# joeylitalien/drmlt-mitsuba

Hardware: AMD Instinct MI355X
Metric: mutations/sec (accepted+rejected) (higher is better)
Workload: dtype f32

## Files before the change

### drmlt-mitsuba_amd/csrc/device_path.h

```cpp
#pragma once
#include "device_bsdf.h"
#include "device_math.h"
#include "device_sampler.h"
#include "device_types.h"

struct Hit {
    int prim;
    float t, u, v;
};

typedef uint32_t u32x4_t __attribute__((ext_vector_type(4)));
template <class T> DEV T load_global16(const T *p) {
    static_assert(sizeof(T) % 16 == 0, "records are read in 16-byte words");
    typedef const u32x4_t __attribute__((address_space(1))) *GQ;
    const GQ q = (GQ) (uintptr_t) p;
    union { T v; u32x4_t w[sizeof(T) / 16]; } u;
#pragma unroll
    for (unsigned i = 0; i < sizeof(T) / 16u; ++i) u.w[i] = q[i];
    return u.v;
}
DEV f3 smooth_record_sum(const DParams &P, float index_bits, float u, float v) {
    typedef float f32x3_t __attribute__((ext_vector_type(3)));
    typedef const char __attribute__((address_space(1))) *GB;
    typedef const f32x3_t __attribute__((address_space(1))) *GQ;
// ... 296 lines not shown
    trav_run<int>(P, T, true, 0);
    return T.h;
}

typedef float float2v __attribute__((ext_vector_type(2)));
typedef const DPrimFlat __attribute__((address_space(4))) *ScalarFlatPtr;

struct FlatRec {
    float2v cx, cy, cz, cw;
    float z0, z1, z2, z3;
    int ks;
};

template <bool TRI> DEV void test_flat(const FlatRec &G, f3 o, f3 d, float tmin, float &best_t, float2v &best_uv, int &best_ks) {
    const float ldz = fmaf(G.z0, d.x, fmaf(G.z1, d.y, G.z2 * d.z));
    const float loz = fmaf(G.z0, o.x, fmaf(G.z1, o.y, fmaf(G.z2, o.z, G.z3)));
    const float t = -loz * fast_rcp(ldz);
    const float2v lo = G.cx * o.x + (G.cy * o.y + (G.cz * o.z + G.cw));
    const float2v ld = G.cx * d.x + (G.cy * d.y + G.cz * d.z);
    const float2v uv = ld * t + lo;
    float w;
    if (TRI && (G.ks & 0xff) == PRIM_TRIANGLE) w = 1.f - (uv.x + uv.y);
    else { const float2v om = 1.f - uv; w = fminf(om.x, om.y); }
    bool hit = fminf(fminf(uv.x, uv.y), w) >= 0.f && t >= tmin && t <= best_t;
    if (TRI) hit = hit && w >= 0.f;
    best_t = hit ? t : best_t;
    best_uv.x = hit ? uv.x : best_uv.x;
    best_uv.y = hit ? uv.y : best_uv.y;
    best_ks = hit ? G.ks : best_ks;
}

#define BOX_FACE_FLAG 0x40000000
typedef const DPrimBox __attribute__((address_space(4))) *ScalarBoxPtr;
struct BoxRec {
    float2v cx, cy, cz, cw;
    float z0, z1, z2, z3;
    uint32_t f0, f1, f2;
};
struct BoxCand { float t, p, q; uint32_t hc; };
DEV BoxCand box_candidate(bool leave, float nx, float ny, float fx, float fy, float tnear, float tfar, float2v lo, float2v ld, float loz, float ldz,
                          uint32_t f0, uint32_t f1, uint32_t f2) {
    BoxCand c;
    c.t = leave ? tfar : tnear;
    const float cx = leave ? fx : nx, cy = leave ? fy : ny;
    const bool a0 = cx == c.t, a1 = cy == c.t;
    const float lda = a0 ? ld.x : (a1 ? ld.y : ldz);
    const uint32_t w = a0 ? f0 : (a1 ? f1 : f2);
    c.hc = ((lda < 0.f) != leave) ? w >> 16 : w & 0xffffu;
    const float2v bxy = ld * c.t + lo;
    const float bzz = fmaf(ldz, c.t, loz);
    c.p = a0 ? bxy.y : bxy.x; c.q = (a0 || a1) ? bzz : bxy.y;
    return c;
}
DEV void test_box(const BoxRec &G, f3 o, f3 d, float tmin, float &best_t, float2v &best_uv, int &best_ks) {
    const uint32_t f0 = G.f0, f1 = G.f1, f2 = G.f2;
    const float ldz = fmaf(G.z0, d.x, fmaf(G.z1, d.y, G.z2 * d.z));
    const float loz = fmaf(G.z0, o.x, fmaf(G.z1, o.y, fmaf(G.z2, o.z, G.z3)));
    const float2v lo = G.cx * o.x + (G.cy * o.y + (G.cz * o.z + G.cw));
    const float2v ld = G.cx * d.x + (G.cy * d.y + G.cz * d.z);
    const float ix = fast_rcp(ld.x), iy = fast_rcp(ld.y), iz = fast_rcp(ldz);
    const float ax = -lo.x * ix, bx = (1.f - lo.x) * ix, ay = -lo.y * iy, by = (1.f - lo.y) * iy, az = -loz * iz, bz = (1.f - loz) * iz;
    const float nx = fminf(ax, bx), fx = fmaxf(ax, bx), ny = fminf(ay, by), fy = fmaxf(ay, by), nz = fminf(az, bz), fz = fmaxf(az, bz);
    const float tnear = fmaxf(fmaxf(nx, ny), nz), tfar = fminf(fminf(fx, fy), fz);
    const bool through = tnear <= tfar && tfar >= tmin && tnear <= best_t;
    const bool inside = !(tnear >= tmin);
    BoxCand c = box_candidate(inside, nx, ny, fx, fy, tnear, tfar, lo, ld, loz, ldz, f0, f1, f2);
    const bool hole = through && !inside && (c.hc & 1u) == 0u;
    if (__ballot(hole)) {
        const BoxCand c2 = box_candidate(true, nx, ny, fx, fy, tnear, tfar, lo, ld, loz, ldz, f0, f1, f2);
        c.t = hole ? c2.t : c.t; c.p = hole ? c2.p : c.p; c.q = hole ? c2.q : c.q; c.hc = hole ? c2.hc : c.hc;
    }
    const bool hit = through && (c.hc & 1u) != 0u && c.t >= tmin && c.t <= best_t;
    best_t = hit ? c.t : best_t;
    best_uv.x = hit ? c.p : best_uv.x;
    best_uv.y = hit ? c.q : best_uv.y;
    best_ks = hit ? (int) (c.hc | BOX_FACE_FLAG) : best_ks;
}

template <bool TRI> DEV Hit trace_flat(const DParams &P, f3 o, f3 d, float tmin, float tmax) {
    ScalarFlatPtr p = (ScalarFlatPtr) (uintptr_t) P.prims_flat;
    auto load = [](ScalarFlatPtr q, FlatRec &G) {
#ifdef DRMLT_FLAT_PLAIN_LOADS
        G.cx = float2v{q->c[0], q->c[1]}; G.cy = float2v{q->c[2], q->c[3]}; G.cz = float2v{q->c[4], q->c[5]}; G.cw = float2v{q->c[6], q->c[7]};
        G.z0 = q->rz[0]; G.z1 = q->rz[1]; G.z2 = q->rz[2]; G.z3 = q->rz[3];
        G.ks = q->kind_shade;
#else
        typedef float f8v __attribute__((ext_vector_type(8)));
        typedef float f4v __attribute__((ext_vector_type(4)));
        const f8v c = *(const volatile f8v __attribute__((address_space(4))) *) &q->c[0];
        const f4v z = *(const volatile f4v __attribute__((address_space(4))) *) &q->rz[0];
        G.ks = *(const volatile int __attribute__((address_space(4))) *) &q->kind_shade;
        G.cx = float2v{c[0], c[1]}; G.cy = float2v{c[2], c[3]}; G.cz = float2v{c[4], c[5]}; G.cw = float2v{c[6], c[7]};
        G.z0 = z[0]; G.z1 = z[1]; G.z2 = z[2]; G.z3 = z[3];
#endif
    };
#define PINF(G) asm volatile("" ::"s"(G.cx.x), "s"(G.cz.x), "s"(G.z0), "s"(G.ks))
    float best_t = tmax;
    float2v best_uv = {0.f, 0.f};
    int best_ks = -1;
    if (P.n_box > 0) {
        auto loadb = [](ScalarBoxPtr q, BoxRec &G) {
            typedef float f8v __attribute__((ext_vector_type(8)));
            typedef float f4v __attribute__((ext_vector_type(4)));
            const f8v c = *(const volatile f8v __attribute__((address_space(4))) *) &q->c[0];
            const f4v z = *(const volatile f4v __attribute__((address_space(4))) *) &q->rz[0];
            typedef const volatile uint32_t __attribute__((address_space(4))) *SU;
            G.f0 = *(SU) &q->fw[0]; G.f1 = *(SU) &q->fw[1]; G.f2 = *(SU) &q->fw[2];
            G.cx = float2v{c[0], c[1]}; G.cy = float2v{c[2], c[3]}; G.cz = float2v{c[4], c[5]}; G.cw = float2v{c[6], c[7]};
            G.z0 = z[0]; G.z1 = z[1]; G.z2 = z[2]; G.z3 = z[3];
        };
        ScalarBoxPtr pb = (ScalarBoxPtr) (uintptr_t) P.prims_box;
        BoxRec A, B;
        loadb(pb, A);
        for (int i = 0; i < P.n_box; i += 2, pb += 2) {
            asm volatile("" ::"s"(A.cx.x), "s"(A.z0), "s"(A.f0));
            loadb(pb + 1, B);
            test_box(A, o, d, tmin, best_t, best_uv, best_ks);
            if (i + 1 < P.n_box) {
                asm volatile("" ::"s"(B.cx.x), "s"(B.z0), "s"(B.f0));
                loadb(pb + 2, A);
                test_box(B, o, d, tmin, best_t, best_uv, best_ks);
            }
        }
    }
    const int n = P.n_flat_rec;
    if (n > 0) {
        FlatRec A, B;
        load(p, A);
        for (int i = 0; i < n; i += 2, p += 2) {
            PINF(A);
            load(p + 1, B);
            test_flat<TRI>(A, o, d, tmin, best_t, best_uv, best_ks);
            if (i + 1 < n) {
                PINF(B);
                load(p + 2, A);
                test_flat<TRI>(B, o, d, tmin, best_t, best_uv, best_ks);
            }
        }
    }
#undef PINF
    Hit h{-1, best_t, best_uv.x, best_uv.y};
    if (best_ks >= 0) {
        if (best_ks & BOX_FACE_FLAG) {
            const uint32_t hc = (uint32_t) best_ks & 0xffffu;
            const float uu = (hc & 2u) ? h.v : h.u, vv = (hc & 2u) ? h.u : h.v;
            h.u = (hc & 4u) ? 1.f - uu : uu;
            h.v = (hc & 8u) ? 1.f - vv : vv;
            best_ks = (int) (((hc >> 4) & 3u) | ((hc >> 6) << 8));
        }
        h.prim = best_ks >> 8;
        if ((best_ks & 0xff) == PRIM_QUAD2) {
            const bool second = h.v > h.u;
            const float uu = second ? h.u : h.u - h.v, vv = second ? h.v - h.u : h.v;
            h.prim += second ? 1 : 0;
            h.u = uu; h.v = vv;
        }
    }
    return h;
}

struct HeldScene {
    BoxRec box[3];
    FlatRec flat;
};
DEV Hit trace_held(const HeldScene &S, uint32_t n_box, uint32_t n_flat, f3 o, f3 d, float tmin, float tmax) {
    float best_t = tmax;
    float2v best_uv = {0.f, 0.f};
    int best_ks = -1;
    if (n_box > 0u) test_box(S.box[0], o, d, tmin, best_t, best_uv, best_ks);
    if (n_box > 1u) test_box(S.box[1], o, d, tmin, best_t, best_uv, best_ks);
    if (n_box > 2u) test_box(S.box[2], o, d, tmin, best_t, best_uv, best_ks);
    if (n_flat > 0u) test_flat<false>(S.flat, o, d, tmin, best_t, best_uv, best_ks);
    Hit h{-1, best_t, best_uv.x, best_uv.y};
    if (best_ks >= 0) {
        if (best_ks & BOX_FACE_FLAG) {
            const uint32_t hc = (uint32_t) best_ks & 0xffffu;
            const float uu = (hc & 2u) ? h.v : h.u, vv = (hc & 2u) ? h.u : h.v;
            h.u = (hc & 4u) ? 1.f - uu : uu;
            h.v = (hc & 8u) ? 1.f - vv : vv;
            best_ks = (int) (((hc >> 4) & 3u) | ((hc >> 6) << 8));
        }
        h.prim = best_ks >> 8;
        if ((best_ks & 0xff) == PRIM_QUAD2) {
            const bool second = h.v > h.u;
            const float uu = second ? h.u : h.u - h.v, vv = second ? h.v - h.u : h.v;
            h.prim += second ? 1 : 0;
            h.u = uu; h.v = vv;
        }
    }
    return h;
}

template <int FEAT = 15> DEV Hit trace(const DParams &P, f3 o, f3 d, float tmin, float tmax, bool any_hit) {
    if ((FEAT & 8) && P.use_bvh) return trace_bvh(P, o, d, tmin, tmax, any_hit);
    if (P.prims_flat) {
        Hit h = P.has_plain_tri ? trace_flat<true>(P, o, d, tmin, tmax) : trace_flat<false>(P, o, d, tmin, tmax);
        if (FEAT & 4)
            for (int i = P.n_flat; i < P.n_prims; ++i) {
                ScalarPrimPtr sp = (ScalarPrimPtr) (uintptr_t) P.prims;
                DPrim G;
#pragma unroll
                for (int k = 0; k < 12; ++k) G.m[k] = sp[i].m[k];
                const int ks = sp[i].kind_shade;
                G.type = PRIM_SPHERE; G.shade = ks >> 8;
                intersect_prim<4>(G, G.shade, o, d, tmin, h);
            }
        return h;
    }
    return trace_brute<FEAT>(P, o, d, tmin, tmax);
}

struct GlobalTables {
    const DShade *sh; const DBsdf *bs; const DEmitter *em;
    DEV DShade shade(int i) const { return load_global16(sh + i); }
    DEV DBsdf bsdf(int i) const { return load_global16(bs + i); }
    DEV DEmitter emitter(int i) const { return load_global16(em + i); }
    DEV float emitter_cdf_lo(int i) const { return load_global_f32(&em[i].cdf_lo); }
    DEV DShade emitter_shade(int, const DEmitter &E) const { return shade(E.prim); }
};
struct LdsTables {
    uint32_t shade_off, bsdf_off, emit_off;
    DEV DShade shade(int i) const {
        const float4 *q = reinterpret_cast<const float4 *>(&lds_x[shade_off + (uint32_t) i * 16u]);
        const float4 a = q[0], b = q[1], c = q[2], d = q[3];
        DShade s;
        s.origin[0] = a.x; s.origin[1] = a.y; s.origin[2] = a.z; s.eu[0] = a.w;
        s.eu[1] = b.x; s.eu[2] = b.y; s.ev[0] = b.z; s.ev[1] = b.w;
        s.ev[2] = c.x; s.n[0] = c.y; s.n[1] = c.z; s.n[2] = c.w;
        s.inv_len_eu = d.x; s.bsdf = __float_as_int(d.y); s.emitter = __float_as_int(d.z); s.inv_area = d.w;
        return s;
    }
    DEV DBsdf bsdf(int i) const {
        const float4 *q = reinterpret_cast<const float4 *>(&lds_x[bsdf_off + (uint32_t) i * 12u]);
        const float4 a = q[0], b = q[1], c = q[2];
        DBsdf r;
        r.type = __float_as_int(a.x); r.rgb[0] = a.y; r.rgb[1] = a.z; r.rgb[2] = a.w;
        r.p[0] = b.x; r.p[1] = b.y; r.p[2] = b.z; r.p[3] = b.w;
        r.p[4] = c.x; r.p[5] = c.y; r.p[6] = c.z; r.p[7] = c.w;
        return r;
    }
    DEV DEmitter emitter(int i) const {
        const float4 *q = reinterpret_cast<const float4 *>(&lds_x[emit_off + (uint32_t) i * 8u]);
        const float4 a = q[0], b = q[1];
        DEmitter e;
        e.radiance[0] = a.x; e.radiance[1] = a.y; e.radiance[2] = a.z; e.prim = __float_as_int(a.w);
        e.cdf_lo = b.x; e.cdf_hi = b.y; e.pad[0] = b.z; e.pad[1] = b.w;
        return e;
    }
    DEV float emitter_cdf_lo(int i) const { return lds_x[emit_off + (uint32_t) i * 8u + 4u]; }
    DEV DShade emitter_shade(int, const DEmitter &E) const { return shade(E.prim); }
    DEV int n_emitters(const DParams &P) const { return P.n_emitters; }
};
struct OneLightTables {
    LdsTables L;
    const DParams &P;
    DEV DShade shade(int i) const { return L.shade(i); }
    DEV DBsdf bsdf(int i) const { return L.bsdf(i); }
    DEV DEmitter emitter(int) const { return P.light; }
    DEV float emitter_cdf_lo(int) const { return P.light.cdf_lo; }
    DEV DShade emitter_shade(int, const DEmitter &) const { DShade s = P.light_shade; asm volatile("" : "+s"(s.inv_area)); return s; }
    DEV constexpr int n_emitters(const DParams &) const { return 1; }
};
struct HeldLightTables {
    LdsTables L;
    const DEmitter &E;
    const DShade &S;
    DEV DShade shade(int i) const { return L.shade(i); }
    DEV DBsdf bsdf(int i) const { return L.bsdf(i); }
    DEV DEmitter emitter(int) const { return E; }
    DEV float emitter_cdf_lo(int) const { return E.cdf_lo; }
    DEV DShade emitter_shade(int, const DEmitter &) const { DShade s = S; s.bsdf = __builtin_amdgcn_readfirstlane(s.bsdf); return s; }
    DEV constexpr int n_emitters(const DParams &) const { return 1; }
};
struct MixedTables {
    const DShade *sh;
    LdsTables L;
    DEV DShade shade(int i) const { return load_global16(sh + i); }
    DEV DBsdf bsdf(int i) const { return L.bsdf(i); }
    DEV DEmitter emitter(int i) const { return L.emitter(i); }
    DEV float emitter_cdf_lo(int i) const { return L.emitter_cdf_lo(i); }
    DEV DShade emitter_shade(int ei, const DEmitter &) const { return L.shade(ei); }
};
struct HybridTables {
    const DShade *sh; const DBsdf *bs; const DEmitter *em;
    LdsTables L;
    bool lds;
    DEV DShade shade(int i) const { return load_global16(sh + i); }
    DEV DBsdf bsdf(int i) const { if (lds) return L.bsdf(i); return load_global16(bs + i); }
    DEV DEmitter emitter(int i) const { if (lds) return L.emitter(i); return load_global16(em + i); }
    DEV float emitter_cdf_lo(int i) const { if (lds) return L.emitter_cdf_lo(i); return load_global_f32(&em[i].cdf_lo); }
    DEV DShade emitter_shade(int ei, const DEmitter &E) const { if (lds) return L.shade(ei); return load_global16(sh + E.prim); }
};
DEV uint32_t small_tables_floats(const DParams &P) { return (uint32_t) P.n_emitters * 16u + (uint32_t) P.n_bsdfs * 12u + (uint32_t) P.n_emitters * 8u; }
DEV void stage_bsdfs_emitters(const DParams &P, const LdsTables &T, uint32_t lane) {
    const float *src = reinterpret_cast<const float *>(P.bsdfs);
    for (uint32_t i = lane; i < (uint32_t) P.n_bsdfs * 12u; i += 64u) lds_x[T.bsdf_off + i] = src[i];
    src = reinterpret_cast<const float *>(P.emitters);
    for (uint32_t i = lane; i < (uint32_t) P.n_emitters * 8u; i += 64u) lds_x[T.emit_off + i] = src[i];
    for (uint32_t i = lane; i < (uint32_t) P.n_emitters * 16u; i += 64u) {
        const int prim = P.emitters[i >> 4].prim;
        lds_x[T.shade_off + i] = reinterpret_cast<const float *>(P.shade + prim)[i & 15u];
    }
}
DEV void stage_tables(const DParams &P, const LdsTables &T, uint32_t lane) {
    const float *src = reinterpret_cast<const float *>(P.shade);
    for (uint32_t i = lane; i < (uint32_t) P.n_shade * 16u; i += 64u) lds_x[T.shade_off + i] = src[i];
    src = reinterpret_cast<const float *>(P.bsdfs);
    for (uint32_t i = lane; i < (uint32_t) P.n_bsdfs * 12u; i += 64u) lds_x[T.bsdf_off + i] = src[i];
    src = reinterpret_cast<const float *>(P.emitters);
    for (uint32_t i = lane; i < (uint32_t) P.n_emitters * 8u; i += 64u) lds_x[T.emit_off + i] = src[i];
}

enum { PH_DONE = 0, PH_BEGIN = 1, PH_CLOSEST = 2, PH_SHADOW = 3, PH_IDLE = 4, PH_FLUSH = 5 };

struct PathState {
    f3 o, d;
    float tmin, tmax;
    f3 thr, Li;
    f3 n, s, wi;
    f3 nee;
    f3 bweight;
    float bpdf, beta_eta, eta;
    float bx, by;
    float px, py;
    int phase, depth, bsdf;
    uint32_t k;
// ... 402 lines not shown
    const float v3 = smp.next(min(k0 + 3u, kmax)), v4 = smp.next(min(k0 + 4u, kmax));
    sr.valid = false;
    f3 Li = ps.Li;
    if (ps.shadow_pending && shadow_clear) Li = Li + ps.nee;
    const bool live = ps.phase != PH_FLUSH && hit.prim >= 0;
    const DShade S = T.shade(hit.prim >= 0 ? hit.prim : 0);
    const f3 p = fma3(ld3(S.eu), hit.u, fma3(ld3(S.ev), hit.v, ld3(S.origin)));
    const f3 n = ld3(S.n);
    const f3 s = ld3(S.eu) * S.inv_len_eu;
    const bool hb = ps.has_bounce;
    const f3 thr_b = hb ? ps.thr * ps.bweight : ps.thr;
    const float eta = hb ? ps.eta * ps.beta_eta : ps.eta;
    if (!RARE_EMITTER_HIT || __ballot(live && hb && S.emitter >= 0 && ps.direct_on && ps.non_specular) != 0ull) {
        const DEmitter E = T.emitter(S.emitter >= 0 ? S.emitter : 0);
        const float dn = dot3(ps.d, n);
        const float dr = dot3(ps.d, ps.n);
        float lumPdf = S.inv_area * hit.t * hit.t / fabsf(dn);
        lumPdf *= E.cdf_hi - E.cdf_lo;
        lumPdf = (!ps.bdelta && dr >= 0.f) ? lumPdf : 0.f;
        const float a = ps.bpdf * ps.bpdf, b = lumPdf * lumPdf;
        const f3 Lm = fma3(thr_b * ld3(E.radiance), a / (a + b), Li);
        if constexpr (RARE_EMITTER_HIT) {
            const bool use = (live & hb & (S.emitter >= 0) & ps.direct_on & ps.non_specular) & (dn < 0.f);
            Li = mk3(use ? Lm.x : Li.x, use ? Lm.y : Li.y, use ? Lm.z : Li.z);
        } else
        if (live && hb && S.emitter >= 0 && ps.direct_on && ps.non_specular && dn < 0.f) Li = Lm;
    }
    const bool want_rr = hb && ps.depth >= P.rr_depth;
    const int depth = hb ? ps.depth + 1 : ps.depth;
    const bool direct_on = hb || ps.direct_on;
    const bool at_max = depth >= P.max_depth && P.max_depth > 0;
    const float rr_q = fminf(max3(thr_b) * eta * eta, 0.95f);
    const bool survives = !want_rr || !(v0 >= rr_q);
    const f3 thr = want_rr ? thr_b * (1.f / rr_q) : thr_b;
    const bool go = live && !at_max && survives;
    const f3 t = cross3(n, s);
    const f3 md = -ps.d;
    const f3 wi = mk3(dot3(md, s), dot3(md, t), dot3(md, n));
    const int bsdf = S.bsdf & 0xffffff;
    const DBsdf B = T.bsdf(bsdf);
    const bool want_nee = direct_on && B.type == 0;
    const float sx0 = want_rr ? v1 : v0, sy = want_rr ? v2 : v1;
    const int bpos = (want_rr ? 1 : 0) + (want_nee ? 2 : 0);
    const float bx = bpos == 0 ? v0 : (bpos == 1 ? v1 : (bpos == 2 ? v2 : v3));
    const float by = bpos == 0 ? v1 : (bpos == 1 ? v2 : (bpos == 2 ? v3 : v4));
    int ei = 0;
    for (int i = 1; i < T.n_emitters(P); ++i)
        if (T.emitter_cdf_lo(i) < sx0) ei = i;
    const DEmitter E = T.emitter(ei);
    const float emPdf = E.cdf_hi - E.cdf_lo;
    const float sx = (sx0 - E.cdf_lo) / emPdf;
    const DShade L = T.emitter_shade(ei, E);
    f3 lp;
    if ((L.bsdf >> 24) == PRIM_RECTANGLE) lp = fma3(ld3(L.eu), sx, fma3(ld3(L.ev), sy, ld3(L.origin)));
    else { const float a = sqrtf(fmaxf(0.f, 1.f - sx)); lp = fma3(ld3(L.eu), 1.f - a, fma3(ld3(L.ev), a * sy, ld3(L.origin))); }
    const f3 ln = ld3(L.n);
    const f3 dv = lp - p;
    const float dist2 = dot3(dv, dv), dist = sqrtf(dist2);
    const f3 dd = dv * (1.f / dist);
    const float dln = dot3(dd, ln);
    const float pdf = dln != 0.f ? L.inv_area * dist2 / fabsf(dln) : 0.f;
    const float drl = dot3(dd, n);
    const f3 wo_l = mk3(dot3(dd, s), dot3(dd, t), dot3(dd, n));
    const f3 bsdfVal = ld3(B.rgb) * (INV_PI_F * wo_l.z);
    const float bsdfPdf = INV_PI_F * wo_l.z;
    const float lpdf = pdf * emPdf;
    const float a = lpdf * lpdf, b = bsdfPdf * bsdfPdf;
    const f3 value = ld3(E.radiance) * (1.f / lpdf);
    const f3 c = thr * value * bsdfVal * (a / (a + b));
    const bool nee = go && want_nee && drl >= 0.f && dln < 0.f && pdf != 0.f && wi.z > 0.f && wo_l.z > 0.f && !is_zero3(c);
    const f3 wo = square_to_cosine_hemisphere(bx, by);
    const f3 bweight = ld3(B.rgb);
    const bool bounce = go && B.type == 0 && wi.z > 0.f && !is_zero3(bweight);
    ps.Li = Li;
    ps.k = k0 + ((live && want_rr) ? 1u : 0u) + (go ? (want_nee ? 4u : 2u) : 0u);
    ps.nrays += (nee ? 1u : 0u) + (bounce ? 1u : 0u);
    ps.shadow_pending = nee;
    ps.phase = bounce ? PH_CLOSEST : (nee ? PH_FLUSH : PH_DONE);
    if (!MASKED || nee) {
        ps.nee = c;
        sr.o = p; sr.d = dd;
        sr.tmin = ray_eps_shadow(p);
        sr.tmax = dist * (1.f - SHADOW_EPSILON_F);
        sr.valid = MASKED || nee;
    }
    if (!MASKED || bounce) {
        ps.thr = thr; ps.eta = eta; ps.depth = depth; ps.direct_on = direct_on;
        ps.wi = wi;
        ps.o = p; ps.n = n; ps.s = s;
        ps.bsdf = bsdf;
        ps.bpdf = INV_PI_F * wo.z;
        ps.bweight = bweight;
        ps.beta_eta = 1.f;
        ps.bdelta = false;
        ps.non_specular = true;
        ps.d = fma3(s, wo.x, fma3(t, wo.y, n * wo.z));
        ps.tmin = ray_eps_closest(p);
        ps.tmax = INFINITY;
        ps.has_bounce = true;
    }
}

template <class SamplerT> DEV DSplat eval_path(const DParams &P, SamplerT &smp, uint32_t &nrays, uint32_t &ndims) {
    PathState ps;
    smp.reset_caches();
    path_init(P, ps);
    Hit h{-1, 0.f, 0.f, 0.f};
// ... 16 lines not shown
```

### drmlt-mitsuba_amd/csrc/kernels.hip

```cpp
#include <algorithm>
#include <cstdlib>
#include <cstdio>
#include <type_traits>
#include "device_path.h"

#include "kernel_common.h"
#include "launch_plan.h"

__device__ __attribute__((noinline)) DSplat eval_boot_sample(const DParams &P, uint32_t index, uint32_t &nd) {
    Sampler smp;
    smp.key0 = P.key0; smp.key1 = P.key1; smp.chain = P.boot_stream; smp.major = index;
    smp.mode = SM_BOOT; smp.arr = nullptr;
    uint32_t nr;
    return eval_path(P, smp, nr, nd);
}

__global__ void __launch_bounds__(64) k_bootstrap(DParams P, uint32_t n, float *lum_out) {
    uint32_t i = blockIdx.x * blockDim.x + threadIdx.x;
    if (i >= n) return;
    uint32_t nd;
    DSplat s = eval_boot_sample(P, i, nd);
    lum_out[i] = s.lum;
    if (P.boot_weighted) { normalize_splat(s, P); lum_out[(size_t) n + i] = s.lum; }
}
// ... 821 lines not shown
#pragma unroll
    for (int i = 0; i < 12; ++i) hold_v(H.cam[i]);
#pragma unroll
    for (int i = 0; i < 3; ++i) {
        hold_v(H.light.radiance[i]); hold_v(H.light_shade.origin[i]); hold_v(H.light_shade.eu[i]); hold_v(H.light_shade.ev[i]); hold_v(H.light_shade.n[i]);
    }
    hold_v(H.light.cdf_lo); hold_v(H.light.cdf_hi); hold_v(H.light_shade.inv_area); hold_v(H.light_shade.bsdf);
}
DEV RowSamplerT<RULE_ORBITAL> w2_sampler(uint32_t key0, uint32_t key1) {
    RowSamplerT<RULE_ORBITAL> s;
    s.key0 = key0; s.key1 = key1;
    s.mode = SM_STAGE1; s.type = 2; s.sigma2 = 0.f;
    s.stride = V4_STRIDE;
    s.x_off = s.y_off = s.xyz = 0u;
    return s;
}
template <bool BOX> DEV void w2_film_put_channel(const DParams &P, const float *lut, float px, float py, float v, int ch) {
    if (P.debug & 1) return;
    float posx = px - 0.5f, posy = py - 0.5f;
    int minx = max((int) ceilf(posx - P.filter_radius), 0), miny = max((int) ceilf(posy - P.filter_radius), 0);
    int maxx = min((int) floorf(posx + P.filter_radius), P.width - 1), maxy = min((int) floorf(posy + P.filter_radius), P.height - 1);
    for (int y = miny; y <= maxy; ++y) {
        const int iy = min((int) fabsf(((float) y - posy) * P.filter_scale), 31);
        float wy = BOX ? (iy < 31 ? P.box_weight : 0.f) : lut[iy];
        for (int x = minx; x <= maxx; ++x) {
            const int ix = min((int) fabsf(((float) x - posx) * P.filter_scale), 31);
            float w = (BOX ? (ix < 31 ? P.box_weight : 0.f) : lut[ix]) * wy;
            atomic_add_global_f32(P.film + ((size_t) y * P.width + x) * 3 + ch, w * v);
        }
    }
}
template <bool BOX> DEV void w2_flush_passes(const DParams &P, const V4Lds &L, const float *lut, uint32_t qn, uint32_t lane) {
    const uint32_t s = lane / 3u, ch = lane - 3u * s;
    for (uint32_t base = 0u; base < qn; base += 21u) {
        const uint32_t e = base + s;
        if (e < qn && s < 21u) {
            const float *q = &lds_x[L.q_off + e];
            w2_film_put_channel<BOX>(P, lut, q[0], q[L.qcap], q[(2u + ch) * L.qcap], (int) ch);
        }
    }
}
DEV void w2_flush(const DParams &P, const V4Lds &L, uint32_t &qn, uint32_t lane) {
    float *const lut = &lds_x[L.list_off];
    if (P.box_weight > 0.f) w2_flush_passes<true>(P, L, lut, qn, lane);
    else if (qn) {
        if (lane < 32u) lut[lane] = P.filter_lut[lane];
        w2_flush_passes<false>(P, L, lut, qn, lane);
    }
    qn = 0u;
}

struct W2HeldScene {
    HeldScene S;
    uint32_t counts;
};
struct W2StreamedScene {};
template <class Rec> DEV void w2_hold_rows(Rec &G, const float *c, const float *rz, bool have) {
    float v[12];
#pragma unroll
    for (int k = 0; k < 12; ++k) v[k] = 0.f;
    if (have) {
#pragma unroll
        for (int k = 0; k < 8; ++k) v[k] = c[k];
#pragma unroll
        for (int k = 0; k < 4; ++k) v[8 + k] = rz[k];
    }
#pragma unroll
    for (int k = 0; k < 12; ++k) hold_v(v[k]);
    G.cx = float2v{v[0], v[1]}; G.cy = float2v{v[2], v[3]}; G.cz = float2v{v[4], v[5]}; G.cw = float2v{v[6], v[7]};
    G.z0 = v[8]; G.z1 = v[9]; G.z2 = v[10]; G.z3 = v[11];
}
DEV W2HeldScene w2_held_scene(const DParams &P) {
    W2HeldScene H;
    const uint32_t n_box = (uint32_t) min(max(P.n_box, 0), 3), n_flat = (uint32_t) min(max(P.n_flat_rec, 0), 1);
#pragma unroll
    for (uint32_t i = 0; i < 3u; ++i) {
        BoxRec &G = H.S.box[i];
        const DPrimBox *q = P.prims_box + i;
        w2_hold_rows(G, q->c, q->rz, i < n_box);
        uint32_t f0 = 0u, f1 = 0u, f2 = 0u;
        if (i < n_box) { f0 = q->fw[0]; f1 = q->fw[1]; f2 = q->fw[2]; }
        hold_v(f0); hold_v(f1); hold_v(f2);
        G.f0 = f0; G.f1 = f1; G.f2 = f2;
    }
    FlatRec &F = H.S.flat;
    w2_hold_rows(F, P.prims_flat->c, P.prims_flat->rz, n_flat > 0u);
    int ks = -1;
    if (n_flat > 0u) ks = P.prims_flat->kind_shade;
    hold_v(ks);
    F.ks = ks;
    H.counts = n_box | (n_flat << 8);
    hold_v(H.counts);
    return H;
}

template <bool HELD> __global__ void __launch_bounds__(CHAIN_BLOCK, 2) k_mutate_w2(DParams P, uint32_t n_mut, uint32_t mut_base) {
    typedef RowSamplerT<RULE_ORBITAL> RowSampler;
    if (threadIdx.x == 0) {
        atomicAdd(P.stats + 14, 1ull); atomicAdd(P.stats + 15, 1ull); atomicAdd(P.stats + 16, 1ull);
        if constexpr (HELD) atomicAdd(P.stats + 17, 1ull);
    }
    const uint32_t lane = threadIdx.x;
    const uint32_t sub = lane & 31u;
    const bool helper = lane >= 32u;
    const uint32_t c = blockIdx.x * 32u + sub;
    const bool live = !helper && c < P.n_chains;
    const uint32_t cc = c < P.n_chains ? c : P.n_chains - 1;
    const uint32_t S = V4_STRIDE;
    int smp_mode = SM_STAGE1;
    uint32_t roles;
    uint32_t qn = 0u;
    ChainState cs;
    float cum = 0.f;
    Counters ct = {0u, 0u, 0u, 0u, 0u};
    PathState ps;
    bool helper_has_ray = false;
    Hit h{-1, 0.f, 0.f, 0.f};
    int batch;
    uint32_t base = 0u, target = 0u, limit = 0u;
    bool reported = false;
    W2Held held = w2_held(P);
    w2_hold(held);
    typename std::conditional<HELD, W2HeldScene, W2StreamedScene>::type scene;
    if constexpr (HELD) scene = w2_held_scene(P);
    uint32_t imp_lo = (uint32_t) (uintptr_t) P.importance, imp_hi = (uint32_t) ((uintptr_t) P.importance >> 32);
    uint32_t done_lo = (uint32_t) (uintptr_t) P.chain_done, done_hi = (uint32_t) ((uintptr_t) P.chain_done >> 32);
    uint32_t left_lo = (uint32_t) (uintptr_t) P.waves_left, left_hi = (uint32_t) ((uintptr_t) P.waves_left >> 32);
    uint32_t key0_v = P.key0, key1_v = P.key1, chain_off_v = P.chain_offset, timid_v = (uint32_t) P.timid_after_large;
    hold_v(imp_lo); hold_v(imp_hi); hold_v(done_lo); hold_v(done_hi); hold_v(left_lo); hold_v(left_hi);
    hold_v(key0_v); hold_v(key1_v); hold_v(chain_off_v); hold_v(timid_v);
    {
        const V4Layout<RULE_ORBITAL> Y = v4_layout<RULE_ORBITAL>(P, V4_QCAP);
        roles = RowSampler::first_roles(Y.group, sub);
        if (!helper) {
            for (uint32_t k = 0; k < Y.D; ++k) lds_x[k * S + sub] = unwrap01(P.x[(size_t) k * P.n_chains + cc]);
            for (uint32_t k = Y.D; k < Y.D4; ++k) lds_x[k * S + sub] = 0.f;
        }
        cs.cur.lum = P.cur_lum[cc]; cs.cur.px = P.cur_px[cc]; cs.cur.py = P.cur_py[cc];
        cs.cur.r = P.cur_r[cc]; cs.cur.g = P.cur_g[cc]; cs.cur.b = P.cur_b[cc];
        cs.y = cs.cur; cs.z = cs.cur;
        cs.a1 = 0.f; cs.coin_acc1 = cs.coin_acc2 = cs.coin_mix = 0.f;
        cs.it = 0u; cs.nd1 = cs.nd2 = 0u; cs.stage = -1; cs.large = false;
        path_init(P, ps);
        base = (P.chain_done && live) ? P.chain_done[cc] : mut_base;
        target = P.chain_done ? n_mut : mut_base + n_mut;
// ... 120 lines not shown
                        const uint32_t ii = valid ? i : 0u;
                        const uint32_t b = (uint32_t) (((float) ii + 0.5f) * rcp_n), j = ii - b * n;
                        const uint32_t cj = (uint32_t) lds_list[j];
                        const uint32_t mj = (uint32_t) __shfl((int) maj_mine, (int) cj, 64);
                        const unsigned inf = (unsigned) __shfl((int) info, (int) cj, 64);
                        smg.set_roles(inf, C.group, cj);
                        const bool coin = b >= nb1;
                        if (valid) {
                            const u4 r = philox4x32_10(Pm.key0, Pm.key1, coin ? 0u : b, coin ? mj + 1u : mj, chain_base_g + cj, coin ? TAG_COIN : TAG_S1);
                            const Unit4 u{{u32_to_unit(r.x), u32_to_unit(r.y), u32_to_unit(r.z), u32_to_unit(r.w)}};
                            if (!coin) row_fill_first_drawn(smg, b, u, (inf & 1u) != 0u);
                            else {
                                float *dst = &lds_x[L.coin_off + cj];
                                dst[0] = u.v[0]; dst[S] = u.v[1]; dst[2u * S] = u.v[2]; dst[3u * S] = u.v[3];
                            }
                        }
                    }
                }
                const uint32_t f2mask = (uint32_t) __ballot(kind == 2);
                if (f2mask) {
                    if (kind == 2) lds_list[__builtin_amdgcn_mbcnt_lo(f2mask, 0u)] = (int) sub;
                    const uint32_t nb2 = Pm.timid_after_large ? D4 / 4u : (D4 / 2u + 3u) / 4u;
                    const uint32_t n = (uint32_t) __popc(f2mask), total = n * nb2;
                    const float rcp_n = 1.f / (float) n;
                    for (uint32_t fb = 0u; fb < total; fb += 64u) {
                        const uint32_t i = fb + lane;
                        const bool valid = i < total;
                        const uint32_t ii = valid ? i : 0u;
                        const uint32_t b = (uint32_t) (((float) ii + 0.5f) * rcp_n), j = ii - b * n;
                        const uint32_t cj = (uint32_t) lds_list[j];
                        const uint32_t mj = (uint32_t) __shfl((int) maj_mine, (int) cj, 64);
                        const unsigned inf = (unsigned) __shfl((int) info, (int) cj, 64);
                        smg.set_roles(inf, C.group, cj);
                        if (valid) smg.fill_second(b, D4, mj, chain_base_g + cj, (inf & 1u) != 0u);
                    }
                }
            }

            if (parked) {
                if (kind == 0) ps.phase = PH_IDLE;
                else {
                    DParams Vb{};
                    Vb.exclude_direct = C.exclude_direct; Vb.width = C.width; Vb.height = C.height;
                    Vb.tan_half_fov = C.tan_half_fov; Vb.inv_aspect = C.inv_aspect; Vb.near_clip = C.near_clip; Vb.far_clip = C.far_clip;
#pragma unroll
                    for (int q = 0; q < 12; ++q) Vb.cam[q] = C.cam[q];
                    smp_mode = smp.mode = cs.stage == 0 ? SM_STAGE1 : SM_STAGE2;
                    path_init(Vb, ps);
                    const float v0 = smp.next(0u), v1 = smp.next(1u);
                    path_begin(Vb, ps, v0, v1);
                }
            }
        }
        const bool tracing = helper ? helper_has_ray : ps.phase == PH_CLOSEST;
        __builtin_amdgcn_s_setprio(0);
        if constexpr (HELD) {
            if (__ballot(tracing)) {
                const uint32_t counts = wave_uniform(scene.counts);
                h = trace_held(scene.S, counts & 0xffu, counts >> 8, ps.o, ps.d, ps.tmin, ps.tmax);
            }
        } else {
            SECTION_PARAMS(Pt);
            if (__ballot(tracing)) h = trace<0>(Pt, ps.o, ps.d, ps.tmin, ps.tmax, helper);
        }
        __builtin_amdgcn_s_setprio(3);
        const unsigned occluded = from_upper_u((helper_has_ray && h.prim >= 0) ? 1u : 0u);
        helper_has_ray = false;
        ShadowRay sr;
        asm volatile("" : "=v"(sr.d.x), "=v"(sr.d.y), "=v"(sr.d.z), "=v"(sr.tmin), "=v"(sr.tmax));
        sr.o = ps.o; sr.valid = false;
        {
            const W2Held &Cs = held;
            if (!helper && ps.phase != PH_DONE && ps.phase != PH_IDLE) {
                RowSampler sms = w2_sampler(0u, 0u);
                sms.set_roles(roles, Cs.group, sub); sms.mode = smp_mode;
                DParams Vs{};
                Vs.eff_dim = Cs.eff_dim; Vs.rr_depth = Cs.rr_depth; Vs.max_depth = Cs.max_depth;
                const LdsTables LT{Cs.shade_off, Cs.bsdf_off, 0u};
                path_step_diffuse<RowSampler, HeldLightTables, false, HELD>(Vs, HeldLightTables{LT, Cs.light, Cs.light_shade}, ps, sms, h, occluded == 0u, sr);
            }
        }
        ps.o.x = lower_keeps(ps.o.x, sr.o.x); ps.o.y = lower_keeps(ps.o.y, sr.o.y); ps.o.z = lower_keeps(ps.o.z, sr.o.z);
        ps.d.x = lower_keeps(ps.d.x, sr.d.x); ps.d.y = lower_keeps(ps.d.y, sr.d.y); ps.d.z = lower_keeps(ps.d.z, sr.d.z);
        ps.tmin = lower_keeps(ps.tmin, sr.tmin); ps.tmax = lower_keeps(ps.tmax, sr.tmax);
        helper_has_ray = lower_keeps_u(0u, sr.valid ? 1u : 0u) != 0u;
    }
    SECTION_PARAMS(Pe);
    const V4Layout<RULE_ORBITAL> Y = v4_layout<RULE_ORBITAL>(Pe, V4_QCAP);
    if (qn + 32u > Y.L.qcap) w2_flush(Pe, Y.L, qn, lane);
    v4_enqueue(Y.L, qn, live && cum > 0.f, cs.cur.px, cs.cur.py, cs.cur.r * cum, cs.cur.g * cum, cs.cur.b * cum);
    w2_flush(Pe, Y.L, qn, lane);
    if (live) {
        RowSampler smp = Y.smp;
        smp.set_roles(roles, Y.group, sub);
        for (uint32_t k = 0; k < Y.D; ++k) Pe.x[(size_t) k * Pe.n_chains + c] = smp.x(k);
        Pe.cur_lum[c] = cs.cur.lum; Pe.cur_px[c] = cs.cur.px; Pe.cur_py[c] = cs.cur.py;
        Pe.cur_r[c] = cs.cur.r; Pe.cur_g[c] = cs.cur.g; Pe.cur_b[c] = cs.cur.b;
        if (Pe.chain_done) Pe.chain_done[c] = base + cs.it;
    }
    if (Pe.chain_done && !reported && lane == 0) atomicSub(Pe.waves_left, 1u);
    flush_counters(Pe, ct, lane);
    const unsigned long long decided = wave_sum((live && !helper) ? cs.it : 0u);
    if (lane == 0) atomicAdd(Pe.stats + 9, decided);
}

#define V5_STACK32_CAP 25
#ifndef V5_ROWS_MEM_WAVES
#define V5_ROWS_MEM_WAVES 3
#endif
#ifndef V5_ROWS_MEM_STACK32_CAP
#define V5_ROWS_MEM_STACK32_CAP 25
#endif
enum { RS_IDLE = 0, RS_BUSY = 1, RS_DONE = 2 };

struct V5Lds {
    uint32_t coin_off, list_off;
    uint32_t q_off;
    uint32_t pool_off;
    uint32_t ring_off;
    uint32_t status_off;
};
DEV V5Lds v5_layout(uint32_t D, uint32_t qcap, bool coin_rows) {
    V5Lds L;
    L.coin_off = D * 64u;
    L.list_off = L.coin_off + (coin_rows ? 4u * 64u : 0u);
    L.q_off = L.list_off + 64u;
    L.pool_off = L.q_off + 5u * qcap;
    L.ring_off = L.pool_off + 8u * V5_SLOTS;
    L.status_off = L.ring_off + V5_SLOTS / 4u;
    return L;
}

template <int FEAT, bool STACK16, bool OVF, bool STAMPS = false, bool LDS_TABLES = false, bool ROWS_MEM = false>
__global__ void __launch_bounds__(CHAIN_BLOCK, ROWS_MEM ? V5_ROWS_MEM_WAVES : 2) k_mutate_v5(DParams P, uint32_t n_mut, uint32_t mut_base) {
    constexpr bool FLAT = (FEAT & 8) == 0;
    typedef typename std::conditional<ROWS_MEM, RowsMem, RowsLds>::type RowsT;
    typedef PoolRowSampler<RowsT> SamplerT;
    constexpr uint32_t QCAP = (FLAT || STACK16) ? V5_QCAP : V5_QCAP_STACK32;
// ... 552 lines not shown
```

Baseline: 3.373 billion.

## Precompute held-scene flags to skip hole and quad2 work, specialize rectangle light

Replaces the per-trace box/flat counts with a precomputed, wave-uniform flag word. The flags record which boxes have open faces and whether any quad2 primitives exist, so the hole re-test and the quad2 split are skipped when the scene has none. Hit post-processing becomes branch-free selects. In the held path the light type is fixed to rectangle at compile time, the occlusion exchange uses permlane32_swap, and the shadow-ray handoff is reorganised. This adds coupling between setup-time flags and the trace logic. The tracing predicate also changes, which risks mistakes if the assumptions about scene or light type do not hold.

```diff
diff --git a/drmlt-mitsuba_amd/csrc/device_path.h b/drmlt-mitsuba_amd/csrc/device_path.h
--- a/drmlt-mitsuba_amd/csrc/device_path.h
+++ b/drmlt-mitsuba_amd/csrc/device_path.h
@@ -372,7 +372,7 @@
     c.p = a0 ? bxy.y : bxy.x; c.q = (a0 || a1) ? bzz : bxy.y;
     return c;
 }
-DEV void test_box(const BoxRec &G, f3 o, f3 d, float tmin, float &best_t, float2v &best_uv, int &best_ks) {
+template <bool OPEN_KNOWN = false> DEV void test_box(const BoxRec &G, f3 o, f3 d, float tmin, float &best_t, float2v &best_uv, int &best_ks, bool open = true) {
     const uint32_t f0 = G.f0, f1 = G.f1, f2 = G.f2;
     const float ldz = fmaf(G.z0, d.x, fmaf(G.z1, d.y, G.z2 * d.z));
     const float loz = fmaf(G.z0, o.x, fmaf(G.z1, o.y, fmaf(G.z2, o.z, G.z3)));
@@ -385,10 +385,12 @@
     const bool through = tnear <= tfar && tfar >= tmin && tnear <= best_t;
     const bool inside = !(tnear >= tmin);
     BoxCand c = box_candidate(inside, nx, ny, fx, fy, tnear, tfar, lo, ld, loz, ldz, f0, f1, f2);
-    const bool hole = through && !inside && (c.hc & 1u) == 0u;
-    if (__ballot(hole)) {
-        const BoxCand c2 = box_candidate(true, nx, ny, fx, fy, tnear, tfar, lo, ld, loz, ldz, f0, f1, f2);
-        c.t = hole ? c2.t : c.t; c.p = hole ? c2.p : c.p; c.q = hole ? c2.q : c.q; c.hc = hole ? c2.hc : c.hc;
+    if (!OPEN_KNOWN || open) {
+        const bool hole = through && !inside && (c.hc & 1u) == 0u;
+        if (OPEN_KNOWN ? __builtin_amdgcn_ballot_w64(hole) != 0ull : __ballot(hole) != 0ull) {
+            const BoxCand c2 = box_candidate(true, nx, ny, fx, fy, tnear, tfar, lo, ld, loz, ldz, f0, f1, f2);
+            c.t = hole ? c2.t : c.t; c.p = hole ? c2.p : c.p; c.q = hole ? c2.q : c.q; c.hc = hole ? c2.hc : c.hc;
+        }
     }
     const bool hit = through && (c.hc & 1u) != 0u && c.t >= tmin && c.t <= best_t;
     best_t = hit ? c.t : best_t;
@@ -483,32 +485,56 @@
     BoxRec box[3];
     FlatRec flat;
 };
-DEV Hit trace_held(const HeldScene &S, uint32_t n_box, uint32_t n_flat, f3 o, f3 d, float tmin, float tmax) {
+enum { HELD_BOX1 = 1, HELD_BOX2 = 2, HELD_FLAT = 4, HELD_OPEN0 = 8, HELD_OPEN1 = 16, HELD_OPEN2 = 32, HELD_QUAD2 = 64 };
+DEV bool held_half_missing(uint32_t half) { return (half & 1u) == 0u; }
+DEV bool held_half_quad2(uint32_t half) { return (half & 1u) != 0u && ((half >> 4) & 3u) == (uint32_t) PRIM_QUAD2; }
+DEV uint32_t held_box_flags(uint32_t f0, uint32_t f1, uint32_t f2, uint32_t open_bit) {
+    bool open = false, quad2 = false;
+    const uint32_t w[3] = {f0, f1, f2};
+#pragma unroll
+    for (int a = 0; a < 3; ++a) {
+        open = open || held_half_missing(w[a] & 0xffffu) || held_half_missing(w[a] >> 16);
+        quad2 = quad2 || held_half_quad2(w[a] & 0xffffu) || held_half_quad2(w[a] >> 16);
+    }
+    return (open ? open_bit : 0u) | (quad2 ? (uint32_t) HELD_QUAD2 : 0u);
+}
+DEV uint32_t held_flags(const HeldScene &S, uint32_t n_box, uint32_t n_flat) {
+    uint32_t flags = (n_box > 1u ? (uint32_t) HELD_BOX1 : 0u) | (n_box > 2u ? (uint32_t) HELD_BOX2 : 0u) | (n_flat > 0u ? (uint32_t) HELD_FLAT : 0u);
+#pragma unroll
+    for (uint32_t i = 0; i < 3u; ++i)
+        if (i < n_box) flags |= held_box_flags(S.box[i].f0, S.box[i].f1, S.box[i].f2, (uint32_t) HELD_OPEN0 << i);
+    if (n_flat > 0u && (S.flat.ks & 0xff) == PRIM_QUAD2) flags |= (uint32_t) HELD_QUAD2;
+    return flags;
+}
+DEV Hit trace_held(const HeldScene &S, uint32_t flags, f3 o, f3 d, float tmin, float tmax) {
     float best_t = tmax;
     float2v best_uv = {0.f, 0.f};
     int best_ks = -1;
-    if (n_box > 0u) test_box(S.box[0], o, d, tmin, best_t, best_uv, best_ks);
-    if (n_box > 1u) test_box(S.box[1], o, d, tmin, best_t, best_uv, best_ks);
-    if (n_box > 2u) test_box(S.box[2], o, d, tmin, best_t, best_uv, best_ks);
-    if (n_flat > 0u) test_flat<false>(S.flat, o, d, tmin, best_t, best_uv, best_ks);
+    test_box<true>(S.box[0], o, d, tmin, best_t, best_uv, best_ks, (flags & HELD_OPEN0) != 0u);
+    if (__builtin_expect((flags & HELD_BOX1) != 0u, 1)) test_box<true>(S.box[1], o, d, tmin, best_t, best_uv, best_ks, (flags & HELD_OPEN1) != 0u);
+    if (__builtin_expect((flags & HELD_BOX2) != 0u, 1)) test_box<true>(S.box[2], o, d, tmin, best_t, best_uv, best_ks, (flags & HELD_OPEN2) != 0u);
+    if (__builtin_expect((flags & HELD_FLAT) != 0u, 1)) test_flat<false>(S.flat, o, d, tmin, best_t, best_uv, best_ks);
     Hit h{-1, best_t, best_uv.x, best_uv.y};
-    if (best_ks >= 0) {
-        if (best_ks & BOX_FACE_FLAG) {
-            const uint32_t hc = (uint32_t) best_ks & 0xffffu;
-            const float uu = (hc & 2u) ? h.v : h.u, vv = (hc & 2u) ? h.u : h.v;
-            h.u = (hc & 4u) ? 1.f - uu : uu;
-            h.v = (hc & 8u) ? 1.f - vv : vv;
-            best_ks = (int) (((hc >> 4) & 3u) | ((hc >> 6) << 8));
-        }
-        h.prim = best_ks >> 8;
-        if ((best_ks & 0xff) == PRIM_QUAD2) {
-            const bool second = h.v > h.u;
-            const float uu = second ? h.u : h.u - h.v, vv = second ? h.v - h.u : h.v;
-            h.prim += second ? 1 : 0;
-            h.u = uu; h.v = vv;
-        }
+    const bool any = best_ks >= 0;
+    const bool face = any && (best_ks & BOX_FACE_FLAG) != 0;
+    const uint32_t hc = (uint32_t) best_ks & 0xffffu;
+    const float uu = (hc & 2u) ? h.v : h.u, vv = (hc & 2u) ? h.u : h.v;
+    const float fu = (hc & 4u) ? 1.f - uu : uu, fv = (hc & 8u) ? 1.f - vv : vv;
+    h.u = face ? fu : h.u;
+    h.v = face ? fv : h.v;
+    const int ks = face ? (int) (((hc >> 4) & 3u) | ((hc >> 6) << 8)) : best_ks;
+    h.prim = any ? ks >> 8 : -1;
+    if (flags & HELD_QUAD2) {
+        const bool quad2 = any && (ks & 0xff) == PRIM_QUAD2;
+        const bool second = h.v > h.u;
+        const float qu = second ? h.u : h.u - h.v, qv = second ? h.v - h.u : h.v;
+        h.prim += (quad2 && second) ? 1 : 0;
+        h.u = quad2 ? qu : h.u; h.v = quad2 ? qv : h.v;
     }
     return h;
+}
+DEV Hit trace_held(const HeldScene &S, uint32_t n_box, uint32_t n_flat, f3 o, f3 d, float tmin, float tmax) {
+    return trace_held(S, held_flags(S, n_box, n_flat), o, d, tmin, tmax);
 }
 
 template <int FEAT = 15> DEV Hit trace(const DParams &P, f3 o, f3 d, float tmin, float tmax, bool any_hit) {
@@ -581,7 +607,8 @@
     DEV DShade emitter_shade(int, const DEmitter &) const { DShade s = P.light_shade; asm volatile("" : "+s"(s.inv_area)); return s; }
     DEV constexpr int n_emitters(const DParams &) const { return 1; }
 };
-struct HeldLightTables {
+template <bool RECT> struct HeldLightTablesT {
+    static constexpr bool rectangle_light = RECT;
     LdsTables L;
     const DEmitter &E;
     const DShade &S;
@@ -589,9 +616,16 @@
     DEV DBsdf bsdf(int i) const { return L.bsdf(i); }
     DEV DEmitter emitter(int) const { return E; }
     DEV float emitter_cdf_lo(int) const { return E.cdf_lo; }
-    DEV DShade emitter_shade(int, const DEmitter &) const { DShade s = S; s.bsdf = __builtin_amdgcn_readfirstlane(s.bsdf); return s; }
+    DEV DShade emitter_shade(int, const DEmitter &) const {
+        DShade s = S;
+        if constexpr (!RECT) s.bsdf = __builtin_amdgcn_readfirstlane(s.bsdf);
+        return s;
+    }
     DEV constexpr int n_emitters(const DParams &) const { return 1; }
 };
+typedef HeldLightTablesT<false> HeldLightTables;
+template <class T, class = void> struct light_is_rectangle : std::false_type {};
+template <class T> struct light_is_rectangle<T, std::void_t<decltype(T::rectangle_light)>> : std::integral_constant<bool, T::rectangle_light> {};
 struct MixedTables {
     const DShade *sh;
     LdsTables L;
@@ -1100,7 +1134,7 @@
     const float sx = (sx0 - E.cdf_lo) / emPdf;
     const DShade L = T.emitter_shade(ei, E);
     f3 lp;
-    if ((L.bsdf >> 24) == PRIM_RECTANGLE) lp = fma3(ld3(L.eu), sx, fma3(ld3(L.ev), sy, ld3(L.origin)));
+    if (light_is_rectangle<TablesT>::value || (L.bsdf >> 24) == PRIM_RECTANGLE) lp = fma3(ld3(L.eu), sx, fma3(ld3(L.ev), sy, ld3(L.origin)));
     else { const float a = sqrtf(fmaxf(0.f, 1.f - sx)); lp = fma3(ld3(L.eu), 1.f - a, fma3(ld3(L.ev), a * sy, ld3(L.origin))); }
     const f3 ln = ld3(L.n);
     const f3 dv = lp - p;
diff --git a/drmlt-mitsuba_amd/csrc/kernels.hip b/drmlt-mitsuba_amd/csrc/kernels.hip
--- a/drmlt-mitsuba_amd/csrc/kernels.hip
+++ b/drmlt-mitsuba_amd/csrc/kernels.hip
@@ -897,7 +897,7 @@
 
 struct W2HeldScene {
     HeldScene S;
-    uint32_t counts;
+    uint32_t flags;
 };
 struct W2StreamedScene {};
 template <class Rec> DEV void w2_hold_rows(Rec &G, const float *c, const float *rz, bool have) {
@@ -934,8 +934,8 @@
     if (n_flat > 0u) ks = P.prims_flat->kind_shade;
     hold_v(ks);
     F.ks = ks;
-    H.counts = n_box | (n_flat << 8);
-    hold_v(H.counts);
+    H.flags = held_flags(H.S, n_box, n_flat);
+    hold_v(H.flags);
     return H;
 }
 
@@ -1162,19 +1162,21 @@
                 }
             }
         }
-        const bool tracing = helper ? helper_has_ray : ps.phase == PH_CLOSEST;
+        const bool tracing = HELD ? (helper_has_ray || ps.phase == PH_CLOSEST) : (helper ? helper_has_ray : ps.phase == PH_CLOSEST);
         __builtin_amdgcn_s_setprio(0);
         if constexpr (HELD) {
-            if (__ballot(tracing)) {
-                const uint32_t counts = wave_uniform(scene.counts);
-                h = trace_held(scene.S, counts & 0xffu, counts >> 8, ps.o, ps.d, ps.tmin, ps.tmax);
-            }
+            if (__builtin_amdgcn_ballot_w64(tracing) != 0ull) h = trace_held(scene.S, wave_uniform(scene.flags), ps.o, ps.d, ps.tmin, ps.tmax);
         } else {
             SECTION_PARAMS(Pt);
             if (__ballot(tracing)) h = trace<0>(Pt, ps.o, ps.d, ps.tmin, ps.tmax, helper);
         }
         __builtin_amdgcn_s_setprio(3);
-        const unsigned occluded = from_upper_u((helper_has_ray && h.prim >= 0) ? 1u : 0u);
+        unsigned occluded;
+        if constexpr (HELD) {
+            unsigned any_v;
+            asm volatile("" : "=v"(any_v));
+            occluded = __builtin_amdgcn_permlane32_swap((helper_has_ray && h.prim >= 0) ? 1u : 0u, any_v, false, false)[1];
+        } else occluded = from_upper_u((helper_has_ray && h.prim >= 0) ? 1u : 0u);
         helper_has_ray = false;
         ShadowRay sr;
         asm volatile("" : "=v"(sr.d.x), "=v"(sr.d.y), "=v"(sr.d.z), "=v"(sr.tmin), "=v"(sr.tmax));
@@ -1187,13 +1189,27 @@
                 DParams Vs{};
                 Vs.eff_dim = Cs.eff_dim; Vs.rr_depth = Cs.rr_depth; Vs.max_depth = Cs.max_depth;
                 const LdsTables LT{Cs.shade_off, Cs.bsdf_off, 0u};
-                path_step_diffuse<RowSampler, HeldLightTables, false, HELD>(Vs, HeldLightTables{LT, Cs.light, Cs.light_shade}, ps, sms, h, occluded == 0u, sr);
-            }
-        }
+                typedef HeldLightTablesT<HELD> LightTables;
+                path_step_diffuse<RowSampler, LightTables, false, HELD>(Vs, LightTables{LT, Cs.light, Cs.light_shade}, ps, sms, h, occluded == 0u, sr);
+            }
+        }
+        if constexpr (HELD) {
+            unsigned valid01 = sr.valid ? 1u : 0u, kept;
+            hold_v(valid01);
+            asm volatile("" : "=v"(kept));
+            float gx = sr.o.x, gy = sr.o.y, gz = sr.o.z;
+            hold_v(gx); hold_v(gy); hold_v(gz);
+            ps.d.x = lower_keeps(ps.d.x, sr.d.x); ps.d.y = lower_keeps(ps.d.y, sr.d.y); ps.d.z = lower_keeps(ps.d.z, sr.d.z);
+            ps.tmin = lower_keeps(ps.tmin, sr.tmin); ps.tmax = lower_keeps(ps.tmax, sr.tmax);
+            ps.o.x = lower_keeps(ps.o.x, gx); ps.o.y = lower_keeps(ps.o.y, gy); ps.o.z = lower_keeps(ps.o.z, gz);
+            const bool handed = lower_keeps_u(kept, valid01) != 0u;
+            helper_has_ray = helper & handed;
+        } else {
         ps.o.x = lower_keeps(ps.o.x, sr.o.x); ps.o.y = lower_keeps(ps.o.y, sr.o.y); ps.o.z = lower_keeps(ps.o.z, sr.o.z);
         ps.d.x = lower_keeps(ps.d.x, sr.d.x); ps.d.y = lower_keeps(ps.d.y, sr.d.y); ps.d.z = lower_keeps(ps.d.z, sr.d.z);
         ps.tmin = lower_keeps(ps.tmin, sr.tmin); ps.tmax = lower_keeps(ps.tmax, sr.tmax);
         helper_has_ray = lower_keeps_u(0u, sr.valid ? 1u : 0u) != 0u;
+        }
     }
     SECTION_PARAMS(Pe);
     const V4Layout<RULE_ORBITAL> Y = v4_layout<RULE_ORBITAL>(Pe, V4_QCAP);
```

Result: faster. 3.450 billion (median of 6 runs) (+2.3%).
